# VITA-Group/UVC

Hardware: AMD Instinct MI355X
Metric: images/sec UVC Stage-1 step, DeiT-Tiny budget=0.5 (higher is better)
Workload: dtype bf16; 1 GPU; deit_tiny_patch16_224 Stage-1 UVC-train step, budget 0.5, per-GPU batch 512, 224x224x3 synthetic, soft distillation alpha 0.1, block gating on; global_batch=512, parallelism=dp1

## Files before the change

### uvc_amd/csrc/gemm.hip

```cpp
#include <type_traits>
#include "common.h"
#include "../../include/uvc_kernels.h"

template <typename T> struct Mma;
template <> struct Mma<bf16_t> {
  static constexpr int CH = 8;
  static constexpr int KSTEP = 32;
  typedef bf16x8 Frag;
  static __device__ __forceinline__ f32x4 mma(const Frag& a, const Frag& b, f32x4 c) {
    return __builtin_amdgcn_mfma_f32_16x16x32_bf16(a, b, c, 0, 0, 0);
  }
};
template <> struct Mma<float> {
  static constexpr int CH = 4;
  static constexpr int KSTEP = 16;
  typedef f32x4 Frag;
  static __device__ __forceinline__ f32x4 mma(const Frag& a, const Frag& b, f32x4 c) {
#pragma unroll
    for (int j = 0; j < 4; ++j) c = __builtin_amdgcn_mfma_f32_16x16x4f32(a[j], b[j], c, 0, 0, 0);
    return c;
  }
};

template <typename TS, typename T> struct ChunkLoad;
// ... 21 lines not shown
template <typename T> struct OutIO;
template <> struct OutIO<float> {
  static __device__ __forceinline__ void st4(float* p, f32x4 v) { *reinterpret_cast<f32x4*>(p) = v; }
  static __device__ __forceinline__ f32x4 ld4(const float* p) { return *reinterpret_cast<const f32x4*>(p); }
};
template <> struct OutIO<bf16_t> {
  static __device__ __forceinline__ void st4(bf16_t* p, f32x4 v) {
    u32x2 r; r[0] = pack_bf16x2(v[0], v[1]); r[1] = pack_bf16x2(v[2], v[3]);
    *reinterpret_cast<u32x2*>(p) = r;
  }
  static __device__ __forceinline__ f32x4 ld4(const bf16_t* p) {
    const u32x2 r = *reinterpret_cast<const u32x2*>(p);
    f32x4 v; v[0] = __uint_as_float(r[0] << 16); v[1] = __uint_as_float(r[0] & 0xffff0000u);
    v[2] = __uint_as_float(r[1] << 16); v[3] = __uint_as_float(r[1] & 0xffff0000u);
    return v;
  }
};

struct NtArgs {
  const void* A; const void* B; void* C; void* C2;
  const float* bias; const void* R; const void* R2; const void* aux; const float* dptr;
  int M, N, K, lda, ldb, ldc, ldr, ldaux;
  float alpha;
  const float* alpha_ptr;
  const float* ln_gamma; const float* ln_beta; void* ln_out; float* ln_mean; float* ln_rstd; float ln_eps;
  int no_dma;
};

template <typename TC> struct OutVec;
template <> struct OutVec<float> {
  static constexpr int VN = 4;
  static __device__ __forceinline__ void st(float* p, const float* v) { *reinterpret_cast<f32x4*>(p) = f32x4{v[0], v[1], v[2], v[3]}; }
};
template <> struct OutVec<bf16_t> {
  static constexpr int VN = 8;
  static __device__ __forceinline__ void st(bf16_t* p, const float* v) {
    u32x4 r;
    r[0] = pack_bf16x2(v[0], v[1]); r[1] = pack_bf16x2(v[2], v[3]); r[2] = pack_bf16x2(v[4], v[5]); r[3] = pack_bf16x2(v[6], v[7]);
    *reinterpret_cast<u32x4*>(p) = r;
  }
  static __device__ __forceinline__ void st_nt(bf16_t* p, const float* v) {
    u32x4 r;
    r[0] = pack_bf16x2(v[0], v[1]); r[1] = pack_bf16x2(v[2], v[3]); r[2] = pack_bf16x2(v[4], v[5]); r[3] = pack_bf16x2(v[6], v[7]);
    __builtin_nontemporal_store(r, reinterpret_cast<u32x4*>(p));
  }
};
template <typename T, int VN> __device__ __forceinline__ void load_vec(const T* p, float* v);
template <> __device__ __forceinline__ void load_vec<float, 4>(const float* p, float* v) {
  const f32x4 r = *reinterpret_cast<const f32x4*>(p); v[0] = r[0]; v[1] = r[1]; v[2] = r[2]; v[3] = r[3];
}
template <> __device__ __forceinline__ void load_vec<float, 8>(const float* p, float* v) { load_vec<float, 4>(p, v); load_vec<float, 4>(p + 4, v + 4); }
template <> __device__ __forceinline__ void load_vec<bf16_t, 8>(const bf16_t* p, float* v) {
  const u32x4 r = *reinterpret_cast<const u32x4*>(p);
#pragma unroll
  for (int e = 0; e < 4; ++e) { v[2 * e] = __uint_as_float(r[e] << 16); v[2 * e + 1] = __uint_as_float(r[e] & 0xffff0000u); }
}
template <> __device__ __forceinline__ void load_vec<bf16_t, 4>(const bf16_t* p, float* v) {
  const u32x2 r = *reinterpret_cast<const u32x2*>(p);
  v[0] = __uint_as_float(r[0] << 16); v[1] = __uint_as_float(r[0] & 0xffff0000u);
  v[2] = __uint_as_float(r[1] << 16); v[3] = __uint_as_float(r[1] & 0xffff0000u);
}

template <typename TC> struct Resid;
template <> struct Resid<float> {
  typedef u32x4 Raw4;
  static __device__ __forceinline__ Raw4 ld4(const void* base, size_t elem) { return *reinterpret_cast<const u32x4*>(reinterpret_cast<const float*>(base) + elem); }
  static __device__ __forceinline__ f32x4 f4(const Raw4& r) { return __builtin_bit_cast(f32x4, r); }
  static __device__ __forceinline__ void get(const u32x4& r, float* v) { const f32x4 f = __builtin_bit_cast(f32x4, r); v[0] = f[0]; v[1] = f[1]; v[2] = f[2]; v[3] = f[3]; }
};
template <> struct Resid<bf16_t> {
  typedef u32x2 Raw4;
  static __device__ __forceinline__ Raw4 ld4(const void* base, size_t elem) { return *reinterpret_cast<const u32x2*>(reinterpret_cast<const bf16_t*>(base) + elem); }
  static __device__ __forceinline__ f32x4 f4(const Raw4& r) {
    return f32x4{__uint_as_float(r[0] << 16), __uint_as_float(r[0] & 0xffff0000u), __uint_as_float(r[1] << 16), __uint_as_float(r[1] & 0xffff0000u)};
  }
  static __device__ __forceinline__ void get(const u32x4& r, float* v) {
#pragma unroll
    for (int e = 0; e < 4; ++e) { v[2 * e] = __uint_as_float(r[e] << 16); v[2 * e + 1] = __uint_as_float(r[e] & 0xffff0000u); }
  }
};

__device__ __forceinline__ float epi_scale_bias(float acc, float alpha, float bias) { return __builtin_fmaf(acc, alpha, bias); }
__device__ __forceinline__ float epi_gate_mix(float v, float r2, float d0, float d1) { return __builtin_fmaf(d1, v, __builtin_fmaf(d0, r2, 0.0f)); }
constexpr int EP_LD = 68;

template <bool SWZ> __device__ __forceinline__ float* stg_at(float* stg, int r, int cg) {
  return SWZ ? stg + r * 64 + ((cg ^ (r & 7)) << 2) : stg + r * EP_LD + (cg << 2);
}
template <typename TC, int EPI> __device__ __forceinline__ void nt_load_bias(const NtArgs& g, int lane, int ncol0, float* bias_v) {
  constexpr int VN = OutVec<TC>::VN, LPR = 64 / VN;
  constexpr bool has_bias = EPI == UVC_EPI_BIAS || EPI == UVC_EPI_BIAS_GELU || EPI == UVC_EPI_BIAS_GELU_OUT || EPI == UVC_EPI_BIAS_RESID ||
                            EPI == UVC_EPI_BIAS_RESID_GATE || EPI == UVC_EPI_BIAS_GELU_GRAD;
  const int n = ncol0 + (lane % LPR) * VN;
#pragma unroll
  for (int e = 0; e < VN; ++e) bias_v[e] = (has_bias && n + e < g.N) ? g.bias[n + e] : 0.f;
}
template <int NIT> struct EpiPre { u32x4 r[NIT], r2[NIT], ax[NIT]; };
template <int EPI> struct EpiOperands {
  static constexpr bool R = EPI == UVC_EPI_BIAS_RESID || EPI == UVC_EPI_BIAS_RESID_GATE, R2 = EPI == UVC_EPI_BIAS_RESID_GATE,
                        AUX = EPI == UVC_EPI_DGELU || EPI == UVC_EPI_MUL_AUX;
  static constexpr int COUNT = (R ? 1 : 0) + (R2 ? 1 : 0) + (AUX ? 1 : 0);
};
template <int EPI, int ROWS>
__device__ __forceinline__ void nt_epilogue_prefetch(const NtArgs& g, int lane, int mrow0, int ncol0, EpiPre<ROWS / 8>& P) {
  const int cc = (lane & 7) * 8, n = ncol0 + cc;
  const bool nfull = (n + 8 <= g.N) && ((g.ldc % 8) == 0);
#pragma unroll
  for (int it = 0; it < ROWS / 8; ++it) {
    const int m = mrow0 + it * 8 + (lane >> 3);
    if (m < g.M && nfull) {
      const size_t mo = (size_t)m;
      if (EpiOperands<EPI>::R && (g.ldr % 8) == 0) P.r[it] = *reinterpret_cast<const u32x4*>(reinterpret_cast<const bf16_t*>(g.R) + mo * g.ldr + n);
      if (EpiOperands<EPI>::R2 && (g.ldr % 8) == 0) P.r2[it] = *reinterpret_cast<const u32x4*>(reinterpret_cast<const bf16_t*>(g.R2) + mo * g.ldr + n);
      if (EpiOperands<EPI>::AUX && (g.ldaux % 8) == 0) P.ax[it] = *reinterpret_cast<const u32x4*>(reinterpret_cast<const bf16_t*>(g.aux) + mo * g.ldaux + n);
    }
  }
}
template <typename T, typename TC, int EPI, int ROWS = 32, bool SWZ = false, bool PRE = false>
__device__ __forceinline__ void nt_epilogue_rows(const NtArgs& g, float* stg, int lane, int mrow0, int ncol0, float alpha, float d0, float d1,
                                                 const float* bias_v, const EpiPre<ROWS / 8>* pre = nullptr) {
  static_assert(!PRE || (sizeof(TC) == 2 && sizeof(T) == 2), "operand prefetch: bf16 C and operands only");
  constexpr int VN = OutVec<TC>::VN;
  constexpr int LPR = 64 / VN;
  constexpr int RPI = 64 / LPR;
  TC* __restrict__ C = reinterpret_cast<TC*>(g.C);
  const int cc = (lane % LPR) * VN;
  const int n = ncol0 + cc;
  const bool nfull = (n + VN <= g.N) && ((g.ldc % VN) == 0);
#pragma unroll
  for (int it = 0; it < ROWS / RPI; ++it) {
    const int r = it * RPI + lane / LPR;
    const int m = mrow0 + r;
    float v[VN];
    load_vec<float, 4>(stg_at<SWZ>(stg, r, cc >> 2), v);
    if (VN == 8) load_vec<float, 4>(stg_at<SWZ>(stg, r, (cc >> 2) + 1), v + 4);
    if (m < g.M && n < g.N) {
      const size_t mo = (size_t)m;
#pragma unroll
      for (int e = 0; e < VN; ++e) v[e] = epi_scale_bias(v[e], alpha, bias_v[e]);
      if (EPI == UVC_EPI_BIAS_GELU_OUT) {
#pragma unroll
        for (int e = 0; e < VN; ++e) v[e] = Gelu<T>::f(v[e]);
      }
      if (EPI == UVC_EPI_BIAS_RESID || EPI == UVC_EPI_BIAS_RESID_GATE) {
        const TC* rp = reinterpret_cast<const TC*>(g.R) + mo * g.ldr + n;
        float rv[VN];
        if (nfull && (g.ldr % VN) == 0) { if constexpr (PRE) Resid<TC>::get(pre->r[it], rv); else load_vec<TC, VN>(rp, rv); }
        else {
#pragma unroll
          for (int e = 0; e < VN; ++e) rv[e] = (n + e < g.N) ? ElemIO<TC>::load(rp + e) : 0.f;
        }
#pragma unroll
        for (int e = 0; e < VN; ++e) v[e] += rv[e];
      }
      if (EPI == UVC_EPI_BIAS_RESID_GATE) {
        const TC* rp = reinterpret_cast<const TC*>(g.R2) + mo * g.ldr + n;
        float rv[VN];
        if (nfull && (g.ldr % VN) == 0) { if constexpr (PRE) Resid<TC>::get(pre->r2[it], rv); else load_vec<TC, VN>(rp, rv); }
        else {
#pragma unroll
          for (int e = 0; e < VN; ++e) rv[e] = (n + e < g.N) ? ElemIO<TC>::load(rp + e) : 0.f;
        }
#pragma unroll
        for (int e = 0; e < VN; ++e) v[e] = epi_gate_mix(v[e], rv[e], d0, d1);
      }
      if (EPI == UVC_EPI_DGELU || EPI == UVC_EPI_MUL_AUX) {
        const T* ap = reinterpret_cast<const T*>(g.aux) + mo * g.ldaux + n;
        float av[VN];
        if (nfull && (g.ldaux % VN) == 0) { if constexpr (PRE) Resid<TC>::get(pre->ax[it], av); else load_vec<T, VN>(ap, av); }
        else {
#pragma unroll
          for (int e = 0; e < VN; ++e) av[e] = (n + e < g.N) ? ElemIO<T>::load(ap + e) : 0.f;
        }
#pragma unroll
        for (int e = 0; e < VN; ++e) v[e] *= (EPI == UVC_EPI_MUL_AUX) ? av[e] : Gelu<T>::g(av[e]);
      }
      float u[VN];
      if (EPI == UVC_EPI_BIAS_GELU_GRAD) {
#pragma unroll
        for (int e = 0; e < VN; ++e) { float fo, go; Gelu<T>::fg(v[e], fo, go); u[e] = fo; v[e] = go; }
      }
      TC* cp = C + mo * g.ldc + n;
      if constexpr (EPI == UVC_EPI_BIAS_GELU_GRAD && sizeof(TC) == 2) { if (nfull) OutVec<TC>::st_nt(cp, v); }
      else
      if (nfull) OutVec<TC>::st(cp, v);
      if (nfull) {}
      else {
#pragma unroll
        for (int e = 0; e < VN; ++e) if (n + e < g.N) ElemIO<TC>::store(cp + e, v[e]);
      }
      if (EPI == UVC_EPI_BIAS_GELU || EPI == UVC_EPI_BIAS_GELU_GRAD) {
        TC* c2 = reinterpret_cast<TC*>(g.C2) + mo * g.ldc + n;
        if (EPI == UVC_EPI_BIAS_GELU) {
#pragma unroll
          for (int e = 0; e < VN; ++e) u[e] = Gelu<T>::f(v[e]);
        }
        if constexpr (EPI == UVC_EPI_BIAS_GELU_GRAD && sizeof(TC) == 2) { if (nfull) OutVec<TC>::st_nt(c2, u); }
        else
        if (nfull) OutVec<TC>::st(c2, u);
        if (nfull) {}
        else {
#pragma unroll
          for (int e = 0; e < VN; ++e) if (n + e < g.N) ElemIO<TC>::store(c2 + e, u[e]);
        }
      }
    }
  }
}

template <typename TA, typename T, typename TC, int EPI>
__global__ __launch_bounds__(256, 2) void k_gemm_nt(NtArgs g) {
  typedef Mma<T> MM;
  constexpr int CH = MM::CH;
  constexpr int BK = 8 * CH;
  __shared__ __attribute__((aligned(16))) char smem[(NT_BM + NT_BN) * NT_ROWB];
  char* sA = smem;
  char* sB = smem + NT_BM * NT_ROWB;
  const TA* __restrict__ A = reinterpret_cast<const TA*>(g.A);
  const T* __restrict__ B = reinterpret_cast<const T*>(g.B);
  const int tid = threadIdx.x, lane = tid & 63, w = tid >> 6;
  const int wm = w >> 1, wn = w & 1;
  const int ntn = (g.N + NT_BN - 1) / NT_BN;
  const int xcd = blockIdx.x & 7, q = blockIdx.x >> 3;
  const int bn = q % ntn, bm = (q / ntn) * 8 + xcd;
  const int m0 = bm * NT_BM, n0 = bn * NT_BN;
  if (m0 >= g.M) return;
  const int lc = tid & 7, lr = tid >> 3;

  u32x4 ra[4], rb[4];
  auto gload = [&](int k0) {
    const int kc = k0 + lc * CH;
#pragma unroll
    for (int i = 0; i < 4; ++i) {
      const int row = lr + 32 * i;
      const int m = m0 + row, n = n0 + row;
      u32x4 z = {0u, 0u, 0u, 0u};
      ra[i] = (m < g.M && kc < g.K) ? ChunkLoad<TA, T>::ld(A + (size_t)m * g.lda + kc) : z;
      rb[i] = (n < g.N && kc < g.K) ? ChunkLoad<T, T>::ld(B + (size_t)n * g.ldb + kc) : z;
    }
  };
  auto lstore = [&]() {
#pragma unroll
    for (int i = 0; i < 4; ++i) {
      const int row = lr + 32 * i;
      *reinterpret_cast<u32x4*>(sA + row * NT_ROWB + lc * 16) = ra[i];
      *reinterpret_cast<u32x4*>(sB + row * NT_ROWB + lc * 16) = rb[i];
    }
  };

  f32x4 acc[4][4];
#pragma unroll
  for (int i = 0; i < 4; ++i)
#pragma unroll
    for (int j = 0; j < 4; ++j) acc[i][j] = f32x4{0.f, 0.f, 0.f, 0.f};

  const int nk = (g.K + BK - 1) / BK;
  gload(0);
  lstore();
  __syncthreads();
  for (int kt = 0; kt < nk; ++kt) {
    if (kt + 1 < nk) gload((kt + 1) * BK);
#pragma unroll
    for (int ks = 0; ks < 2; ++ks) {
      typename MM::Frag fa[4], fb[4];
      const int coff = (ks * 4 + (lane >> 4)) * 16;
#pragma unroll
      for (int i = 0; i < 4; ++i) fa[i] = lds_frag<T>(sA + (wm * 64 + i * 16 + (lane & 15)) * NT_ROWB + coff);
#pragma unroll
      for (int j = 0; j < 4; ++j) fb[j] = lds_frag<T>(sB + (wn * 64 + j * 16 + (lane & 15)) * NT_ROWB + coff);
#pragma unroll
      for (int i = 0; i < 4; ++i)
#pragma unroll
        for (int j = 0; j < 4; ++j) acc[i][j] = MM::mma(fb[j], fa[i], acc[i][j]);
    }
    if (kt + 1 < nk) {
      __syncthreads();
      lstore();
      __syncthreads();
    }
  }

  float alpha = g.alpha;
  if (g.alpha_ptr) alpha *= *g.alpha_ptr;
  float d0 = 0.f, d1 = 1.f;
  if (EPI == UVC_EPI_BIAS_RESID_GATE) { d0 = g.dptr[0]; d1 = g.dptr[1]; }
  float* stg = reinterpret_cast<float*>(smem) + w * (32 * EP_LD);
  float bias_v[OutVec<TC>::VN];
  nt_load_bias<TC, EPI>(g, lane, n0 + wn * 64, bias_v);
  __syncthreads();
#pragma unroll
  for (int h = 0; h < 2; ++h) {
#pragma unroll
    for (int ii = 0; ii < 2; ++ii)
#pragma unroll
      for (int j = 0; j < 4; ++j)
        *reinterpret_cast<f32x4*>(stg + (ii * 16 + (lane & 15)) * EP_LD + j * 16 + (lane >> 4) * 4) = acc[2 * h + ii][j];
    __syncthreads();
    nt_epilogue_rows<T, TC, EPI>(g, stg, lane, m0 + wm * 64 + h * 32, n0 + wn * 64, alpha, d0, d1, bias_v);
    __syncthreads();
  }
}

constexpr int WS_BM = 64;

template <typename TA, typename TC, int EPI, int KT, int WS_NW, int NJ = 4>
__global__ __launch_bounds__(64 * WS_NW, (KT > 6 && WS_NW > 6) ? 1 : (NJ == 4 || KT > 6) ? 2 : 4) void k_gemm_ws(NtArgs g, int ngroups, int nslots) {
  typedef bf16_t T;
  typedef Mma<T> MM;
  constexpr int ROWB = KT * 64 + 32;
  constexpr int CPR = KT * 4;
  constexpr int NLD = (WS_BM * CPR + 64 * WS_NW - 1) / (64 * WS_NW);
  constexpr int CW = 16 * NJ, EPW = CW + 4;
  constexpr int VN = OutVec<TC>::VN, LPR = CW / VN, RPI = 64 / LPR;
  constexpr bool DYN = KT > 6;
  constexpr int IMGB = WS_BM * ROWB;
  extern __shared__ __attribute__((aligned(16))) char ws_dyn[];
  __shared__ __attribute__((aligned(16))) char sA_st[DYN ? 16 : 2 * IMGB];
  __shared__ __attribute__((aligned(16))) float sStage_st[DYN ? 4 : WS_NW * 16 * EPW];
  char* const sAb = DYN ? ws_dyn : sA_st;
  float* const sStg = DYN ? reinterpret_cast<float*>(ws_dyn + 2 * IMGB) : sStage_st;
  const int tid = threadIdx.x, lane = tid & 63, w = tid >> 6, gq = lane >> 4, li = lane & 15;
  const int L = blockIdx.x;
  const int grp = (L >> 3) % ngroups, slot = (L / (8 * ngroups)) * 8 + (L & 7);
  const int n0 = grp * CW * WS_NW + w * CW;
  const bool active = n0 < g.N;
  const TA* __restrict__ A = reinterpret_cast<const TA*>(g.A);
  const T* __restrict__ W = reinterpret_cast<const T*>(g.B);
  TC* __restrict__ C = reinterpret_cast<TC*>(g.C);
  const int ntiles = (g.M + WS_BM - 1) / WS_BM;

  typename MM::Frag bf[NJ][KT];
  if (active) {
#pragma unroll
    for (int j = 0; j < NJ; ++j)
#pragma unroll
      for (int ks = 0; ks < KT; ++ks)
        bf[j][ks] = __builtin_bit_cast(typename MM::Frag, *reinterpret_cast<const u32x4*>(W + (size_t)(n0 + j * 16 + li) * g.ldb + (ks * 4 + gq) * 8));
  }
  float alpha = g.alpha;
  if (g.alpha_ptr) alpha *= *g.alpha_ptr;
  float d0 = 0.f, d1 = 1.f;
  if (EPI == UVC_EPI_BIAS_RESID_GATE) { d0 = g.dptr[0]; d1 = g.dptr[1]; }
  const int cc = (lane % LPR) * VN;
  const int n = n0 + cc;
  float bias_v[VN];
#pragma unroll
  for (int e = 0; e < VN; ++e) bias_v[e] = 0.f;
  if (active && (EPI == UVC_EPI_BIAS || EPI == UVC_EPI_BIAS_GELU || EPI == UVC_EPI_BIAS_GELU_OUT || EPI == UVC_EPI_BIAS_RESID || EPI == UVC_EPI_BIAS_RESID_GATE ||
                 EPI == UVC_EPI_BIAS_GELU_GRAD || EPI == UVC_EPI_BIAS_GELU_GRAD_Q8)) {
#pragma unroll
    for (int e = 0; e < VN; ++e) bias_v[e] = g.bias[n + e];
  }

  u32x4 ra[NLD];
  auto gload = [&](int tile) {
    const int m0 = tile * WS_BM;
    const u32x4 z = {0u, 0u, 0u, 0u};
#pragma unroll
    for (int i = 0; i < NLD; ++i) {
      const int id = tid + 64 * WS_NW * i, row = id / CPR, c = id % CPR;
      const int m = m0 + row;
      ra[i] = (row < WS_BM && m < g.M) ? ChunkLoad<TA, T>::ld(A + (size_t)m * g.lda + c * 8) : z;
    }
  };
  auto lstore = [&](int buf) {
#pragma unroll
    for (int i = 0; i < NLD; ++i) {
      const int id = tid + 64 * WS_NW * i, row = id / CPR, c = id % CPR;
      if (row < WS_BM) *reinterpret_cast<u32x4*>(sAb + buf * IMGB + row * ROWB + c * 16) = ra[i];
    }
  };

  constexpr int IT = 16 / RPI;
  struct Epi { u32x4 r[IT]; u32x4 r2[IT]; u32x4 ax[IT]; };
  auto eload = [&](Epi& E, int tile_, int sub_) {
    if (!active) return;
#pragma unroll
    for (int it = 0; it < IT; ++it) {
      const int m = tile_ * WS_BM + sub_ * 16 + it * RPI + lane / LPR;
      const bool ok = m < g.M && tile_ < ntiles;
      const size_t mo = (size_t)(ok ? m : 0);
      if (EPI == UVC_EPI_BIAS_RESID || EPI == UVC_EPI_BIAS_RESID_GATE) E.r[it] = *reinterpret_cast<const u32x4*>(reinterpret_cast<const TC*>(g.R) + mo * g.ldr + n);
      if (EPI == UVC_EPI_BIAS_RESID_GATE) E.r2[it] = *reinterpret_cast<const u32x4*>(reinterpret_cast<const TC*>(g.R2) + mo * g.ldr + n);
      if (EPI == UVC_EPI_DGELU || EPI == UVC_EPI_MUL_AUX) E.ax[it] = *reinterpret_cast<const u32x4*>(reinterpret_cast<const T*>(g.aux) + mo * g.ldaux + n);
      if (EPI == UVC_EPI_MUL_AUX_Q8) {
        const u32x2 q = *reinterpret_cast<const u32x2*>(reinterpret_cast<const unsigned char*>(g.aux) + mo * g.ldaux + n);
        E.ax[it][0] = q[0]; E.ax[it][1] = q[1];
      }
    }
  };
  auto subtile = [&](int buf_, int m0_, int sub_, const Epi& E) {
    if (!active) return;
    float* stg = sStg + w * (16 * EPW);
    {
      typename MM::Frag fa[KT];
#pragma unroll
      for (int ks = 0; ks < KT; ++ks) fa[ks] = lds_frag<T>(sAb + buf_ * IMGB + (sub_ * 16 + li) * ROWB + (ks * 4 + gq) * 16);
#pragma unroll
      for (int j = 0; j < NJ; ++j) {
        f32x4 c = {0.f, 0.f, 0.f, 0.f};
#pragma unroll
        for (int ks = 0; ks < KT; ++ks) c = MM::mma(bf[j][ks], fa[ks], c);
        *reinterpret_cast<f32x4*>(stg + li * EPW + j * 16 + gq * 4) = c;
      }
    }
    __builtin_amdgcn_wave_barrier();
    unsigned qc[IT][2];
#pragma unroll
    for (int it = 0; it < IT; ++it) { qc[it][0] = 0u; qc[it][1] = 0u; }
#pragma unroll
    for (int it = 0; it < IT; ++it) {
      const int r = it * RPI + lane / LPR;
      const int m = m0_ + sub_ * 16 + r;
      float v[VN];
      load_vec<float, VN>(stg + r * EPW + cc, v);
      if (m < g.M) {
        const size_t mo = (size_t)m;
#pragma unroll
        for (int e = 0; e < VN; ++e) v[e] = epi_scale_bias(v[e], alpha, bias_v[e]);
        if (EPI == UVC_EPI_BIAS_RESID || EPI == UVC_EPI_BIAS_RESID_GATE) {
          float rv[VN];
          Resid<TC>::get(E.r[it], rv);
#pragma unroll
          for (int e = 0; e < VN; ++e) v[e] += rv[e];
        }
        if (EPI == UVC_EPI_BIAS_RESID_GATE) {
          float rv[VN];
          Resid<TC>::get(E.r2[it], rv);
#pragma unroll
          for (int e = 0; e < VN; ++e) v[e] = epi_gate_mix(v[e], rv[e], d0, d1);
        }
        if (EPI == UVC_EPI_DGELU) {
#pragma unroll
          for (int e = 0; e < 4; ++e) {
            v[2 * e] *= Gelu<T>::g(__uint_as_float(E.ax[it][e] << 16));
            v[2 * e + 1] *= Gelu<T>::g(__uint_as_float(E.ax[it][e] & 0xffff0000u));
          }
        }
        if (EPI == UVC_EPI_MUL_AUX) {
#pragma unroll
          for (int e = 0; e < 4; ++e) {
            v[2 * e] *= __uint_as_float(E.ax[it][e] << 16);
            v[2 * e + 1] *= __uint_as_float(E.ax[it][e] & 0xffff0000u);
          }
        }
        if constexpr (EPI == UVC_EPI_MUL_AUX_Q8) {
          static_assert(VN == 8, "q8 epilogue: bf16 C");
#pragma unroll
          for (int e = 0; e < 8; ++e)
            v[e] *= __builtin_fmaf((float)((E.ax[it][e >> 2] >> (8 * (e & 3))) & 0xffu), UVC_Q8_STEP, UVC_Q8_LO);
        }
        if (EPI == UVC_EPI_BIAS_GELU_OUT) {
#pragma unroll
          for (int e = 0; e < VN; ++e) v[e] = Gelu<T>::f(v[e]);
        }
        float u[VN];
        if (EPI == UVC_EPI_BIAS_GELU_GRAD || EPI == UVC_EPI_BIAS_GELU_GRAD_Q8) {
#pragma unroll
          for (int e = 0; e < VN; ++e) { float fo, go; Gelu<T>::fg(v[e], fo, go); u[e] = fo; v[e] = go; }
        }
        if constexpr (EPI == UVC_EPI_BIAS_GELU_GRAD_Q8) {
          static_assert(VN == 8, "q8 epilogue: bf16 C2");
          unsigned qw[2] = {0u, 0u};
#pragma unroll
          for (int e = 0; e < 8; ++e)
            qw[e >> 2] = __builtin_amdgcn_cvt_pk_u8_f32(__builtin_fmaf(v[e], 1.0f / UVC_Q8_STEP, -UVC_Q8_LO / UVC_Q8_STEP), e & 3, qw[e >> 2]);
          qc[it][0] = qw[0]; qc[it][1] = qw[1];
          OutVec<TC>::st_nt(reinterpret_cast<TC*>(g.C2) + mo * g.ldc + n, u);
        } else {
        if constexpr (EPI == UVC_EPI_BIAS_GELU_GRAD && sizeof(TC) == 2 && KT == 6) OutVec<TC>::st_nt(C + mo * g.ldc + n, v);
        else
        OutVec<TC>::st(C + mo * g.ldc + n, v);
        if (EPI == UVC_EPI_BIAS_GELU || EPI == UVC_EPI_BIAS_GELU_GRAD) {
          if (EPI == UVC_EPI_BIAS_GELU) {
#pragma unroll
            for (int e = 0; e < VN; ++e) u[e] = Gelu<T>::f(v[e]);
          }
          if constexpr (EPI == UVC_EPI_BIAS_GELU_GRAD && sizeof(TC) == 2 && KT == 6) OutVec<TC>::st_nt(reinterpret_cast<TC*>(g.C2) + mo * g.ldc + n, u);
          else
          OutVec<TC>::st(reinterpret_cast<TC*>(g.C2) + mo * g.ldc + n, u);
        }
        }
      }
    }
    if constexpr (EPI == UVC_EPI_BIAS_GELU_GRAD_Q8) {
      const bool odd = lane & 1;
      if constexpr (IT == 2) {
        static_assert(LPR == 8 && RPI == 8, "q8 epilogue: four waves x 64 columns");
        const unsigned s0 = odd ? qc[0][0] : qc[1][0], s1 = odd ? qc[0][1] : qc[1][1];
        const unsigned r0 = (unsigned)__builtin_amdgcn_mov_dpp((int)s0, 0xB1, 0xF, 0xF, true);
        const unsigned r1 = (unsigned)__builtin_amdgcn_mov_dpp((int)s1, 0xB1, 0xF, 0xF, true);
        const int m = m0_ + sub_ * 16 + (odd ? RPI : 0) + lane / LPR;
        if (m < g.M) {
          const u32x4 o = odd ? u32x4{r0, r1, qc[1][0], qc[1][1]} : u32x4{qc[0][0], qc[0][1], r0, r1};
          __builtin_nontemporal_store(o, reinterpret_cast<u32x4*>(reinterpret_cast<unsigned char*>(g.C) + (size_t)m * g.ldc + (n & ~15)));
        }
      } else {
        static_assert(IT == 1 && LPR == 4, "q8 epilogue: eight waves x 32 columns");
        const unsigned r0 = (unsigned)__builtin_amdgcn_mov_dpp((int)qc[0][0], 0xB1, 0xF, 0xF, true);
        const unsigned r1 = (unsigned)__builtin_amdgcn_mov_dpp((int)qc[0][1], 0xB1, 0xF, 0xF, true);
        const int m = m0_ + sub_ * 16 + lane / LPR;
        if (m < g.M && !odd)
          __builtin_nontemporal_store(u32x4{qc[0][0], qc[0][1], r0, r1}, reinterpret_cast<u32x4*>(reinterpret_cast<unsigned char*>(g.C) + (size_t)m * g.ldc + n));
      }
    }
    __builtin_amdgcn_wave_barrier();
  };

  int tile = slot;
  if (tile >= ntiles) return;
  Epi E0, E1;
  gload(tile);
  eload(E0, tile, 0);
  lstore(0);
  __syncthreads();
  int buf = 0;
  for (; tile < ntiles; tile += nslots) {
    const int next = tile + nslots;
    if (next < ntiles) gload(next);
    const int m0 = tile * WS_BM;
    eload(E1, tile, 1);
    subtile(buf, m0, 0, E0);
    eload(E0, tile, 2);
    subtile(buf, m0, 1, E1);
    eload(E1, tile, 3);
    subtile(buf, m0, 2, E0);
    eload(E0, next, 0);
    subtile(buf, m0, 3, E1);
    if (next < ntiles) lstore(buf ^ 1);
    __syncthreads();
    buf ^= 1;
  }
}

static bool ws_ok(const NtArgs& a, int vn) {
  return (a.K == 192 || a.K == 128) && a.N % 64 == 0 && a.ldb == a.K && a.lda % 8 == 0 && a.ldc % vn == 0 && a.ldr % vn == 0 &&
         a.ldaux % vn == 0 && a.M >= 4096;
}
template <typename TA, typename TC, int KT, int WS_NW>
static int launch_ws_epi(const NtArgs& a, int epi, hipStream_t st) {
  const int ngroups = ceil_div(a.N, 64 * WS_NW);
  const int ntiles = ceil_div(a.M, WS_BM);
#ifndef UVC_WS_WG_TOTAL
#define UVC_WS_WG_TOTAL 512
#endif
  int nslots = (UVC_WS_WG_TOTAL / ngroups) & ~7;
  if (nslots < 8) nslots = 8;
  if (nslots > ((ntiles + 7) & ~7)) nslots = (ntiles + 7) & ~7;
  const int grid = nslots * ngroups;
  if (epi == UVC_EPI_BIAS_GELU_GRAD_Q8) {
    if constexpr (sizeof(TA) == 2 && sizeof(TC) == 2 && KT == 6 && WS_NW == 4) {
      k_gemm_ws<TA, TC, UVC_EPI_BIAS_GELU_GRAD_Q8, KT, WS_NW><<<grid, 64 * WS_NW, 0, st>>>(a, ngroups, nslots);
      UVC_CHECK_LAUNCH();
      return UVC_OK;
    } else return uvc_set_error_msg(UVC_ERR_UNSUPPORTED, "uvc_gemm_nt: UVC_EPI_BIAS_GELU_GRAD_Q8 outside uvc_gemm_nt_q8_supported");
  }
#define WS_CASE(E) case E: k_gemm_ws<TA, TC, E, KT, WS_NW><<<grid, 64 * WS_NW, 0, st>>>(a, ngroups, nslots); break;
  switch (epi) {
    WS_CASE(UVC_EPI_NONE) WS_CASE(UVC_EPI_BIAS) WS_CASE(UVC_EPI_BIAS_GELU) WS_CASE(UVC_EPI_BIAS_RESID)
    WS_CASE(UVC_EPI_BIAS_RESID_GATE) WS_CASE(UVC_EPI_DGELU) WS_CASE(UVC_EPI_BIAS_GELU_OUT) WS_CASE(UVC_EPI_BIAS_GELU_GRAD) WS_CASE(UVC_EPI_MUL_AUX)
    default: return uvc_set_error_msg(UVC_ERR_ARG, "uvc_gemm_nt: unknown epilogue");
  }
#undef WS_CASE
  UVC_CHECK_LAUNCH();
  return UVC_OK;
}
static bool ws384_ok(const NtArgs& a, int epi, int vn, bool a_f32) {
  if (epi == UVC_EPI_DGELU) return false;
  if (epi == UVC_EPI_NONE && !(vn == 8 && a.N % 128 == 0 && a.N >= 512)) return false;
  return !a_f32 && a.K == 384 && a.N % 192 == 0 && a.ldb == a.K && a.lda % 8 == 0 && a.ldc % vn == 0 && a.ldr % vn == 0 && a.ldaux % vn == 0 && a.M >= 4096;
}
template <typename TC, int NW = 6>
static int launch_ws384(const NtArgs& a, int epi, hipStream_t st) {
  constexpr int KT = 12, NJ = 2;
  const int ngroups = ceil_div(a.N, 32 * NW);
  const int ntiles = ceil_div(a.M, WS_BM);
  int nslots = (256 / ngroups) & ~7;
  if (nslots < 8) nslots = 8;
  if (nslots > ((ntiles + 7) & ~7)) nslots = (ntiles + 7) & ~7;
  const int grid = nslots * ngroups;
  const int sh = 2 * WS_BM * (KT * 64 + 32) + NW * 16 * (16 * NJ + 4) * 4;
#define WS_CASE(E) case E: { \
    UVC_MAX_LDS(sh, k_gemm_ws<bf16_t, TC, E, KT, NW, NJ>); \
    k_gemm_ws<bf16_t, TC, E, KT, NW, NJ><<<grid, 64 * NW, sh, st>>>(a, ngroups, nslots); } break;
  switch (epi) {
    WS_CASE(UVC_EPI_NONE) WS_CASE(UVC_EPI_BIAS) WS_CASE(UVC_EPI_BIAS_GELU) WS_CASE(UVC_EPI_BIAS_RESID)
    WS_CASE(UVC_EPI_BIAS_RESID_GATE) WS_CASE(UVC_EPI_BIAS_GELU_OUT) WS_CASE(UVC_EPI_BIAS_GELU_GRAD) WS_CASE(UVC_EPI_MUL_AUX)
    default: return uvc_set_error_msg(UVC_ERR_ARG, "uvc_gemm_nt: unknown epilogue");
  }
#undef WS_CASE
  UVC_CHECK_LAUNCH();
  return UVC_OK;
}

template <typename TA, typename TC, int KT>
static int launch_ws_narrow(const NtArgs& a, int epi, hipStream_t st) {
  const int ngroups = ceil_div(a.N, 256);
  const int ntiles = ceil_div(a.M, WS_BM);
  int nslots = (UVC_WS_WG_TOTAL / ngroups) & ~7;
  if (nslots < 8) nslots = 8;
  if (nslots > ((ntiles + 7) & ~7)) nslots = (ntiles + 7) & ~7;
  const int grid = nslots * ngroups;
#define WS_CASE(E) case E: k_gemm_ws<TA, TC, E, KT, 8, 2><<<grid, 512, 0, st>>>(a, ngroups, nslots); break;
  switch (epi) {
    WS_CASE(UVC_EPI_DGELU) WS_CASE(UVC_EPI_MUL_AUX) WS_CASE(UVC_EPI_MUL_AUX_Q8) WS_CASE(UVC_EPI_BIAS_GELU_GRAD_Q8)
    default: return uvc_set_error_msg(UVC_ERR_ARG, "uvc_gemm_nt: epilogue");
  }
#undef WS_CASE
  UVC_CHECK_LAUNCH();
  return UVC_OK;
}
template <typename TA, typename TC>
static int launch_ws(const NtArgs& a, int epi, hipStream_t st) {
  if constexpr (sizeof(TC) == 2 && sizeof(TA) == 2) {
    if (a.N % 256 == 0 && a.K == 192 && (epi == UVC_EPI_DGELU || epi == UVC_EPI_MUL_AUX || epi == UVC_EPI_MUL_AUX_Q8)) return launch_ws_narrow<TA, TC, 6>(a, epi, st);
#ifdef UVC_FC1_NARROW
    if (a.N % 256 == 0 && a.K == 192 && epi == UVC_EPI_BIAS_GELU_GRAD_Q8) return launch_ws_narrow<TA, TC, 6>(a, epi, st);
#endif
  }
  if (epi == UVC_EPI_MUL_AUX_Q8) return uvc_set_error_msg(UVC_ERR_UNSUPPORTED, "uvc_gemm_nt: UVC_EPI_MUL_AUX_Q8 outside uvc_gemm_nt_q8_supported");
  if (a.N % 256 == 0) return a.K == 192 ? launch_ws_epi<TA, TC, 6, 4>(a, epi, st) : launch_ws_epi<TA, TC, 4, 4>(a, epi, st);
  return a.K == 192 ? launch_ws_epi<TA, TC, 6, 3>(a, epi, st) : launch_ws_epi<TA, TC, 4, 3>(a, epi, st);
}

constexpr int WN_BM = 32;

template <typename TC, int EPI, int KT>
__global__ __launch_bounds__(768) void k_gemm_wsn(NtArgs g) {
  typedef bf16_t T;
  typedef Mma<T> MM;
  constexpr int K = KT * 32, NTH = 768;
  constexpr int ROWB = K * 2 + 32, CPR = K / 8;
  constexpr int NLD = (WN_BM * CPR + NTH - 1) / NTH;
  constexpr bool RES = EPI == UVC_EPI_BIAS_RESID || EPI == UVC_EPI_BIAS_RESID_GATE;
  extern __shared__ __attribute__((aligned(16))) char smem[];
  char* sA0 = smem;
  char* sA1 = smem + WN_BM * ROWB;
  const int tid = threadIdx.x, lane = tid & 63, w = tid >> 6, gq = lane >> 4, li = lane & 15;
  const T* __restrict__ A = reinterpret_cast<const T*>(g.A);
  const T* __restrict__ W = reinterpret_cast<const T*>(g.B);
  TC* __restrict__ C = reinterpret_cast<TC*>(g.C);
  const int ntiles = (g.M + WN_BM - 1) / WN_BM;
  const int n = w * 16 + gq * 4;

  typename MM::Frag bf[KT];
#pragma unroll
  for (int ks = 0; ks < KT; ++ks)
    bf[ks] = __builtin_bit_cast(typename MM::Frag, *reinterpret_cast<const u32x4*>(W + (size_t)(w * 16 + li) * g.ldb + (ks * 4 + gq) * 8));
  float alpha = g.alpha;
  if (g.alpha_ptr) alpha *= *g.alpha_ptr;
  float d0 = 0.f, d1 = 1.f;
  if (EPI == UVC_EPI_BIAS_RESID_GATE) { d0 = g.dptr[0]; d1 = g.dptr[1]; }
  f32x4 bias4 = {0.f, 0.f, 0.f, 0.f};
  if (EPI == UVC_EPI_BIAS || RES) bias4 = *reinterpret_cast<const f32x4*>(g.bias + n);

  u32x4 ra[NLD];
  auto gload = [&](int tile) {
    const int m0 = tile * WN_BM;
    const u32x4 z = {0u, 0u, 0u, 0u};
#pragma unroll
    for (int i = 0; i < NLD; ++i) {
      const int id = tid + NTH * i, row = id / CPR, c = id % CPR;
      const int m = m0 + row;
      ra[i] = (row < WN_BM && m < g.M) ? *reinterpret_cast<const u32x4*>(A + (size_t)m * g.lda + c * 8) : z;
    }
  };
  auto lstore = [&](char* buf) {
#pragma unroll
    for (int i = 0; i < NLD; ++i) {
      const int id = tid + NTH * i, row = id / CPR, c = id % CPR;
      if (row < WN_BM) *reinterpret_cast<u32x4*>(buf + row * ROWB + c * 16) = ra[i];
    }
  };
  struct Epi { f32x4 r[2]; f32x4 r2[2]; };
  auto eload = [&](Epi& E, int tile_) {
    if (!RES) return;
#pragma unroll
    for (int s2 = 0; s2 < 2; ++s2) {
      const int m = tile_ * WN_BM + s2 * 16 + li;
      const size_t off = (m < g.M && tile_ < ntiles) ? (size_t)m * g.ldr + n : 0;
      E.r[s2] = Resid<TC>::f4(Resid<TC>::ld4(g.R, off));
      if (EPI == UVC_EPI_BIAS_RESID_GATE) E.r2[s2] = Resid<TC>::f4(Resid<TC>::ld4(g.R2, off));
    }
  };

  int tile = blockIdx.x;
  if (tile >= ntiles) return;
  Epi E, En;
  gload(tile);
  eload(E, tile);
  lstore(sA0);
  __syncthreads();
  int par = 0;
  for (; tile < ntiles; tile += gridDim.x) {
    const int next = tile + gridDim.x;
    if (next < ntiles) gload(next);
    const char* buf = par ? sA1 : sA0;
    f32x4 c0 = {0.f, 0.f, 0.f, 0.f}, c1 = {0.f, 0.f, 0.f, 0.f};
#pragma unroll
    for (int ks = 0; ks < KT; ++ks) {
      const typename MM::Frag f0 = lds_frag<T>(buf + li * ROWB + (ks * 4 + gq) * 16);
      const typename MM::Frag f1 = lds_frag<T>(buf + (16 + li) * ROWB + (ks * 4 + gq) * 16);
      c0 = MM::mma(bf[ks], f0, c0);
      c1 = MM::mma(bf[ks], f1, c1);
    }
    eload(En, next);
#pragma unroll
    for (int s2 = 0; s2 < 2; ++s2) {
      const int m = tile * WN_BM + s2 * 16 + li;
      f32x4 v = s2 ? c1 : c0;
      if (m < g.M) {
        float o[4];
#pragma unroll
        for (int e = 0; e < 4; ++e) o[e] = epi_scale_bias(v[e], alpha, bias4[e]);
        if (RES) {
#pragma unroll
          for (int e = 0; e < 4; ++e) o[e] += E.r[s2][e];
        }
        if (EPI == UVC_EPI_BIAS_RESID_GATE) {
#pragma unroll
          for (int e = 0; e < 4; ++e) o[e] = epi_gate_mix(o[e], E.r2[s2][e], d0, d1);
        }
        if (sizeof(TC) == 4) *reinterpret_cast<f32x4*>(reinterpret_cast<float*>(C) + (size_t)m * g.ldc + n) = f32x4{o[0], o[1], o[2], o[3]};
        else { u32x2 q; q[0] = pack_bf16x2(o[0], o[1]); q[1] = pack_bf16x2(o[2], o[3]); *reinterpret_cast<u32x2*>(reinterpret_cast<bf16_t*>(C) + (size_t)m * g.ldc + n) = q; }
      }
    }
    E = En;
    if (next < ntiles) lstore(par ? sA0 : sA1);
    __syncthreads();
    par ^= 1;
  }
}

template <typename TC, int EPI, int KT>
__global__ __launch_bounds__(768) void k_gemm_wsn16(NtArgs g) {
  typedef bf16_t T;
  typedef Mma<T> MM;
  constexpr int K = KT * 32, NTH = 768;
  constexpr int ROWB = K * 2 + 32, CPR = K / 8;
  constexpr int NLD = (16 * CPR + NTH - 1) / NTH;
  constexpr bool RES = EPI == UVC_EPI_BIAS_RESID || EPI == UVC_EPI_BIAS_RESID_GATE;
  extern __shared__ __attribute__((aligned(16))) char smem[];
  char* sA0 = smem;
  char* sA1 = smem + 16 * ROWB;
  const int tid = threadIdx.x, lane = tid & 63, w = tid >> 6, gq = lane >> 4, li = lane & 15;
  const T* __restrict__ A = reinterpret_cast<const T*>(g.A);
  const T* __restrict__ W = reinterpret_cast<const T*>(g.B);
  TC* __restrict__ C = reinterpret_cast<TC*>(g.C);
  const int ntiles = (g.M + 16 - 1) / 16;
  const int n = w * 16 + gq * 4;

  typename MM::Frag bf[KT];
#pragma unroll
  for (int ks = 0; ks < KT; ++ks)
    bf[ks] = __builtin_bit_cast(typename MM::Frag, *reinterpret_cast<const u32x4*>(W + (size_t)(w * 16 + li) * g.ldb + (ks * 4 + gq) * 8));
  float alpha = g.alpha;
  if (g.alpha_ptr) alpha *= *g.alpha_ptr;
  float d0 = 0.f, d1 = 1.f;
  if (EPI == UVC_EPI_BIAS_RESID_GATE) { d0 = g.dptr[0]; d1 = g.dptr[1]; }
  f32x4 bias4 = {0.f, 0.f, 0.f, 0.f};
  if (EPI == UVC_EPI_BIAS || RES) bias4 = *reinterpret_cast<const f32x4*>(g.bias + n);

  u32x4 ra[NLD];
  auto gload = [&](int tile) {
    const int m0 = tile * 16;
    const u32x4 z = {0u, 0u, 0u, 0u};
#pragma unroll
    for (int i = 0; i < NLD; ++i) {
      const int id = tid + NTH * i, row = id / CPR, c = id % CPR;
      const int m = m0 + row;
      ra[i] = (row < 16 && m < g.M) ? *reinterpret_cast<const u32x4*>(A + (size_t)m * g.lda + c * 8) : z;
    }
  };
  auto lstore = [&](char* buf) {
#pragma unroll
    for (int i = 0; i < NLD; ++i) {
      const int id = tid + NTH * i, row = id / CPR, c = id % CPR;
      if (row < 16) *reinterpret_cast<u32x4*>(buf + row * ROWB + c * 16) = ra[i];
    }
  };
  struct Epi { typename Resid<TC>::Raw4 r[1]; typename Resid<TC>::Raw4 r2[1]; };
  auto eload = [&](Epi& E, int tile_) {
    if (!RES) return;
#pragma unroll
    for (int s2 = 0; s2 < 1; ++s2) {
      const int m = tile_ * 16 + s2 * 16 + li;
      const size_t off = (m < g.M && tile_ < ntiles) ? (size_t)m * g.ldr + n : 0;
      E.r[s2] = Resid<TC>::ld4(g.R, off);
      if (EPI == UVC_EPI_BIAS_RESID_GATE) E.r2[s2] = Resid<TC>::ld4(g.R2, off);
    }
  };

  int tile = blockIdx.x;
  if (tile >= ntiles) return;
  Epi E, En;
  gload(tile);
  eload(E, tile);
  lstore(sA0);
  __syncthreads();
  int par = 0;
  for (; tile < ntiles; tile += gridDim.x) {
    const int next = tile + gridDim.x;
    if (next < ntiles) gload(next);
    const char* buf = par ? sA1 : sA0;
    f32x4 c0 = {0.f, 0.f, 0.f, 0.f};
#pragma unroll
    for (int ks = 0; ks < KT; ++ks) c0 = MM::mma(bf[ks], lds_frag<T>(buf + li * ROWB + (ks * 4 + gq) * 16), c0);
    eload(En, next);
#pragma unroll
    for (int s2 = 0; s2 < 1; ++s2) {
      const int m = tile * 16 + s2 * 16 + li;
      f32x4 v = c0;
      if (m < g.M) {
        float o[4];
#pragma unroll
        for (int e = 0; e < 4; ++e) o[e] = epi_scale_bias(v[e], alpha, bias4[e]);
        if (RES) {
          const f32x4 rv = Resid<TC>::f4(E.r[s2]);
#pragma unroll
          for (int e = 0; e < 4; ++e) o[e] += rv[e];
        }
        if (EPI == UVC_EPI_BIAS_RESID_GATE) {
          const f32x4 rv = Resid<TC>::f4(E.r2[s2]);
#pragma unroll
          for (int e = 0; e < 4; ++e) o[e] = epi_gate_mix(o[e], rv[e], d0, d1);
        }
        if (sizeof(TC) == 4) *reinterpret_cast<f32x4*>(reinterpret_cast<float*>(C) + (size_t)m * g.ldc + n) = f32x4{o[0], o[1], o[2], o[3]};
        else { u32x2 q; q[0] = pack_bf16x2(o[0], o[1]); q[1] = pack_bf16x2(o[2], o[3]); *reinterpret_cast<u32x2*>(reinterpret_cast<bf16_t*>(C) + (size_t)m * g.ldc + n) = q; }
      }
    }
    E = En;
    if (next < ntiles) lstore(par ? sA0 : sA1);
    __syncthreads();
// ... 2366 lines not shown
```

Baseline: 47230 images/sec.

## Add full-tile fast path and optional MMA/epilogue software pipeline in weight-stationary GEMM

Restructures the weight-stationary GEMM loop into mma and epilogue lambdas. A compile-time full-tile path drops per-row bounds checks for non-operand epilogues and uses 32-bit row offsets from a precomputed base pointer. An optional pipeline, UVC_WS_PIPE (off by default), overlaps the next subtile's MFMAs with the current GELU epilogue using scheduling group barriers. The fast path adds template instantiations and code size, and the 32-bit offset arithmetic assumes row offsets within a tile fit in unsigned.

```diff
diff --git a/uvc_amd/csrc/gemm.hip b/uvc_amd/csrc/gemm.hip
--- a/uvc_amd/csrc/gemm.hip
+++ b/uvc_amd/csrc/gemm.hip
@@ -347,6 +347,7 @@
 }
 
 constexpr int WS_BM = 64;
+__device__ __forceinline__ char* ws_sbase(const void* p, size_t off) { return reinterpret_cast<char*>(const_cast<void*>(p)) + off; }
 
 template <typename TA, typename TC, int EPI, int KT, int WS_NW, int NJ = 4>
 __global__ __launch_bounds__(64 * WS_NW, (KT > 6 && WS_NW > 6) ? 1 : (NJ == 4 || KT > 6) ? 2 : 4) void k_gemm_ws(NtArgs g, int ngroups, int nslots) {
@@ -417,12 +418,23 @@
   };
 
   constexpr int IT = 16 / RPI;
+#ifndef UVC_WS_PIPE
+#define UVC_WS_PIPE 0
+#endif
+  constexpr bool OPERANDS = EPI == UVC_EPI_BIAS_RESID || EPI == UVC_EPI_BIAS_RESID_GATE || EPI == UVC_EPI_DGELU || EPI == UVC_EPI_MUL_AUX || EPI == UVC_EPI_MUL_AUX_Q8;
+  constexpr bool GELU_EPI = EPI == UVC_EPI_BIAS_GELU || EPI == UVC_EPI_BIAS_GELU_OUT || EPI == UVC_EPI_BIAS_GELU_GRAD || EPI == UVC_EPI_BIAS_GELU_GRAD_Q8;
+  constexpr bool PIPE = UVC_WS_PIPE && KT == 6 && NJ == 4 && GELU_EPI;
+  constexpr bool FAST = !OPERANDS || (NJ == 2 && KT == 6 && (EPI == UVC_EPI_MUL_AUX || EPI == UVC_EPI_MUL_AUX_Q8));
+  constexpr int VPM = 6;
   struct Epi { u32x4 r[IT]; u32x4 r2[IT]; u32x4 ax[IT]; };
+  Epi E0, E1;
+  const int lrow = lane / LPR;
+  const unsigned loC = (unsigned)(lrow * g.ldc + n) * (unsigned)sizeof(TC);
   auto eload = [&](Epi& E, int tile_, int sub_) {
     if (!active) return;
 #pragma unroll
     for (int it = 0; it < IT; ++it) {
-      const int m = tile_ * WS_BM + sub_ * 16 + it * RPI + lane / LPR;
+      const int m = tile_ * WS_BM + sub_ * 16 + it * RPI + lrow;
       const bool ok = m < g.M && tile_ < ntiles;
       const size_t mo = (size_t)(ok ? m : 0);
       if (EPI == UVC_EPI_BIAS_RESID || EPI == UVC_EPI_BIAS_RESID_GATE) E.r[it] = *reinterpret_cast<const u32x4*>(reinterpret_cast<const TC*>(g.R) + mo * g.ldr + n);
@@ -434,146 +446,187 @@
       }
     }
   };
-  auto subtile = [&](int buf_, int m0_, int sub_, const Epi& E) {
-    if (!active) return;
-    float* stg = sStg + w * (16 * EPW);
-    {
-      typename MM::Frag fa[KT];
-#pragma unroll
-      for (int ks = 0; ks < KT; ++ks) fa[ks] = lds_frag<T>(sAb + buf_ * IMGB + (sub_ * 16 + li) * ROWB + (ks * 4 + gq) * 16);
-#pragma unroll
-      for (int j = 0; j < NJ; ++j) {
-        f32x4 c = {0.f, 0.f, 0.f, 0.f};
-#pragma unroll
-        for (int ks = 0; ks < KT; ++ks) c = MM::mma(bf[j][ks], fa[ks], c);
-        *reinterpret_cast<f32x4*>(stg + li * EPW + j * 16 + gq * 4) = c;
-      }
-    }
-    __builtin_amdgcn_wave_barrier();
+  float* const stg = sStg + w * (16 * EPW);
+  f32x4 acc[NJ];
+  auto mma_sub = [&](int buf_, int sub_) {
+    typename MM::Frag fa[KT];
+#pragma unroll
+    for (int ks = 0; ks < KT; ++ks) fa[ks] = lds_frag<T>(sAb + buf_ * IMGB + (sub_ * 16 + li) * ROWB + (ks * 4 + gq) * 16);
+#pragma unroll
+    for (int j = 0; j < NJ; ++j) {
+      f32x4 c = {0.f, 0.f, 0.f, 0.f};
+#pragma unroll
+      for (int ks = 0; ks < KT; ++ks) c = MM::mma(bf[j][ks], fa[ks], c);
+      if constexpr (PIPE) acc[j] = c;
+      else *reinterpret_cast<f32x4*>(stg + li * EPW + j * 16 + gq * 4) = c;
+    }
+  };
+  auto epilogue = [&](auto full_c, int m0_, int sub_, const Epi& E, const float (&v)[IT][VN]) {
+    constexpr bool FULL = decltype(full_c)::value;
     unsigned qc[IT][2];
 #pragma unroll
     for (int it = 0; it < IT; ++it) { qc[it][0] = 0u; qc[it][1] = 0u; }
 #pragma unroll
     for (int it = 0; it < IT; ++it) {
-      const int r = it * RPI + lane / LPR;
-      const int m = m0_ + sub_ * 16 + r;
-      float v[VN];
-      load_vec<float, VN>(stg + r * EPW + cc, v);
-      if (m < g.M) {
-        const size_t mo = (size_t)m;
-#pragma unroll
-        for (int e = 0; e < VN; ++e) v[e] = epi_scale_bias(v[e], alpha, bias_v[e]);
+      const int rb = m0_ + sub_ * 16 + it * RPI;
+      const bool ok = FULL || rb + lrow < g.M;
+      TC* const cp = reinterpret_cast<TC*>(ws_sbase(C, (size_t)rb * (size_t)g.ldc * sizeof(TC)) + (size_t)loC);
+      TC* const c2p = reinterpret_cast<TC*>(ws_sbase(g.C2, (size_t)rb * (size_t)g.ldc * sizeof(TC)) + (size_t)loC);
+      float vv[VN];
+      if constexpr (PIPE) {
+#pragma unroll
+        for (int e = 0; e < VN; ++e) vv[e] = v[it][e];
+      } else load_vec<float, VN>(stg + (it * RPI + lrow) * EPW + cc, vv);
+      if (ok) {
+#pragma unroll
+        for (int e = 0; e < VN; ++e) vv[e] = epi_scale_bias(vv[e], alpha, bias_v[e]);
         if (EPI == UVC_EPI_BIAS_RESID || EPI == UVC_EPI_BIAS_RESID_GATE) {
           float rv[VN];
           Resid<TC>::get(E.r[it], rv);
 #pragma unroll
-          for (int e = 0; e < VN; ++e) v[e] += rv[e];
+          for (int e = 0; e < VN; ++e) vv[e] += rv[e];
         }
         if (EPI == UVC_EPI_BIAS_RESID_GATE) {
           float rv[VN];
           Resid<TC>::get(E.r2[it], rv);
 #pragma unroll
-          for (int e = 0; e < VN; ++e) v[e] = epi_gate_mix(v[e], rv[e], d0, d1);
+          for (int e = 0; e < VN; ++e) vv[e] = epi_gate_mix(vv[e], rv[e], d0, d1);
         }
         if (EPI == UVC_EPI_DGELU) {
 #pragma unroll
           for (int e = 0; e < 4; ++e) {
-            v[2 * e] *= Gelu<T>::g(__uint_as_float(E.ax[it][e] << 16));
-            v[2 * e + 1] *= Gelu<T>::g(__uint_as_float(E.ax[it][e] & 0xffff0000u));
+            vv[2 * e] *= Gelu<T>::g(__uint_as_float(E.ax[it][e] << 16));
+            vv[2 * e + 1] *= Gelu<T>::g(__uint_as_float(E.ax[it][e] & 0xffff0000u));
           }
         }
         if (EPI == UVC_EPI_MUL_AUX) {
 #pragma unroll
           for (int e = 0; e < 4; ++e) {
-            v[2 * e] *= __uint_as_float(E.ax[it][e] << 16);
-            v[2 * e + 1] *= __uint_as_float(E.ax[it][e] & 0xffff0000u);
+            vv[2 * e] *= __uint_as_float(E.ax[it][e] << 16);
+            vv[2 * e + 1] *= __uint_as_float(E.ax[it][e] & 0xffff0000u);
           }
         }
         if constexpr (EPI == UVC_EPI_MUL_AUX_Q8) {
           static_assert(VN == 8, "q8 epilogue: bf16 C");
 #pragma unroll
           for (int e = 0; e < 8; ++e)
-            v[e] *= __builtin_fmaf((float)((E.ax[it][e >> 2] >> (8 * (e & 3))) & 0xffu), UVC_Q8_STEP, UVC_Q8_LO);
+            vv[e] *= __builtin_fmaf((float)((E.ax[it][e >> 2] >> (8 * (e & 3))) & 0xffu), UVC_Q8_STEP, UVC_Q8_LO);
         }
         if (EPI == UVC_EPI_BIAS_GELU_OUT) {
 #pragma unroll
-          for (int e = 0; e < VN; ++e) v[e] = Gelu<T>::f(v[e]);
+          for (int e = 0; e < VN; ++e) vv[e] = Gelu<T>::f(vv[e]);
         }
         float u[VN];
         if (EPI == UVC_EPI_BIAS_GELU_GRAD || EPI == UVC_EPI_BIAS_GELU_GRAD_Q8) {
 #pragma unroll
-          for (int e = 0; e < VN; ++e) { float fo, go; Gelu<T>::fg(v[e], fo, go); u[e] = fo; v[e] = go; }
+          for (int e = 0; e < VN; ++e) { float fo, go; Gelu<T>::fg(vv[e], fo, go); u[e] = fo; vv[e] = go; }
         }
         if constexpr (EPI == UVC_EPI_BIAS_GELU_GRAD_Q8) {
           static_assert(VN == 8, "q8 epilogue: bf16 C2");
           unsigned qw[2] = {0u, 0u};
 #pragma unroll
           for (int e = 0; e < 8; ++e)
-            qw[e >> 2] = __builtin_amdgcn_cvt_pk_u8_f32(__builtin_fmaf(v[e], 1.0f / UVC_Q8_STEP, -UVC_Q8_LO / UVC_Q8_STEP), e & 3, qw[e >> 2]);
+            qw[e >> 2] = __builtin_amdgcn_cvt_pk_u8_f32(__builtin_fmaf(vv[e], 1.0f / UVC_Q8_STEP, -UVC_Q8_LO / UVC_Q8_STEP), e & 3, qw[e >> 2]);
           qc[it][0] = qw[0]; qc[it][1] = qw[1];
-          OutVec<TC>::st_nt(reinterpret_cast<TC*>(g.C2) + mo * g.ldc + n, u);
+          if (ok) OutVec<TC>::st_nt(c2p, u);
         } else {
-        if constexpr (EPI == UVC_EPI_BIAS_GELU_GRAD && sizeof(TC) == 2 && KT == 6) OutVec<TC>::st_nt(C + mo * g.ldc + n, v);
+        if constexpr (EPI == UVC_EPI_BIAS_GELU_GRAD && sizeof(TC) == 2 && KT == 6) { if (ok) OutVec<TC>::st_nt(cp, vv); }
         else
-        OutVec<TC>::st(C + mo * g.ldc + n, v);
+        { if (ok) OutVec<TC>::st(cp, vv); }
         if (EPI == UVC_EPI_BIAS_GELU || EPI == UVC_EPI_BIAS_GELU_GRAD) {
           if (EPI == UVC_EPI_BIAS_GELU) {
 #pragma unroll
-            for (int e = 0; e < VN; ++e) u[e] = Gelu<T>::f(v[e]);
+            for (int e = 0; e < VN; ++e) u[e] = Gelu<T>::f(vv[e]);
           }
-          if constexpr (EPI == UVC_EPI_BIAS_GELU_GRAD && sizeof(TC) == 2 && KT == 6) OutVec<TC>::st_nt(reinterpret_cast<TC*>(g.C2) + mo * g.ldc + n, u);
+          if constexpr (EPI == UVC_EPI_BIAS_GELU_GRAD && sizeof(TC) == 2 && KT == 6) { if (ok) OutVec<TC>::st_nt(c2p, u); }
           else
-          OutVec<TC>::st(reinterpret_cast<TC*>(g.C2) + mo * g.ldc + n, u);
+          { if (ok) OutVec<TC>::st(c2p, u); }
         }
         }
       }
     }
     if constexpr (EPI == UVC_EPI_BIAS_GELU_GRAD_Q8) {
       const bool odd = lane & 1;
+      unsigned char* const qp = reinterpret_cast<unsigned char*>(ws_sbase(g.C, (size_t)(m0_ + sub_ * 16) * (size_t)g.ldc));
       if constexpr (IT == 2) {
         static_assert(LPR == 8 && RPI == 8, "q8 epilogue: four waves x 64 columns");
         const unsigned s0 = odd ? qc[0][0] : qc[1][0], s1 = odd ? qc[0][1] : qc[1][1];
         const unsigned r0 = (unsigned)__builtin_amdgcn_mov_dpp((int)s0, 0xB1, 0xF, 0xF, true);
         const unsigned r1 = (unsigned)__builtin_amdgcn_mov_dpp((int)s1, 0xB1, 0xF, 0xF, true);
-        const int m = m0_ + sub_ * 16 + (odd ? RPI : 0) + lane / LPR;
-        if (m < g.M) {
+        const int mr = (odd ? RPI : 0) + lrow;
+        if (FULL || m0_ + sub_ * 16 + mr < g.M) {
           const u32x4 o = odd ? u32x4{r0, r1, qc[1][0], qc[1][1]} : u32x4{qc[0][0], qc[0][1], r0, r1};
-          __builtin_nontemporal_store(o, reinterpret_cast<u32x4*>(reinterpret_cast<unsigned char*>(g.C) + (size_t)m * g.ldc + (n & ~15)));
+          __builtin_nontemporal_store(o, reinterpret_cast<u32x4*>(qp + (size_t)(unsigned)(mr * g.ldc + (n & ~15))));
         }
       } else {
         static_assert(IT == 1 && LPR == 4, "q8 epilogue: eight waves x 32 columns");
         const unsigned r0 = (unsigned)__builtin_amdgcn_mov_dpp((int)qc[0][0], 0xB1, 0xF, 0xF, true);
         const unsigned r1 = (unsigned)__builtin_amdgcn_mov_dpp((int)qc[0][1], 0xB1, 0xF, 0xF, true);
-        const int m = m0_ + sub_ * 16 + lane / LPR;
-        if (m < g.M && !odd)
-          __builtin_nontemporal_store(u32x4{qc[0][0], qc[0][1], r0, r1}, reinterpret_cast<u32x4*>(reinterpret_cast<unsigned char*>(g.C) + (size_t)m * g.ldc + n));
-      }
+        if ((FULL || m0_ + sub_ * 16 + lrow < g.M) && !odd)
+          __builtin_nontemporal_store(u32x4{qc[0][0], qc[0][1], r0, r1}, reinterpret_cast<u32x4*>(qp + (size_t)(unsigned)(lrow * g.ldc + n)));
+      }
+    }
+  };
+  auto subtile = [&](auto full_c, int buf_, int m0_, int sub_, const Epi& E, int nbuf, int nsub) {
+    if (!active) return;
+    if constexpr (!PIPE) mma_sub(buf_, sub_);
+    else {
+#pragma unroll
+      for (int j = 0; j < NJ; ++j) *reinterpret_cast<f32x4*>(stg + li * EPW + j * 16 + gq * 4) = acc[j];
     }
     __builtin_amdgcn_wave_barrier();
+    float v[IT][VN];
+    if constexpr (PIPE) {
+#pragma unroll
+      for (int it = 0; it < IT; ++it) load_vec<float, VN>(stg + (it * RPI + lrow) * EPW + cc, v[it]);
+      __builtin_amdgcn_wave_barrier();
+      mma_sub(nbuf, nsub);
+    }
+    epilogue(full_c, m0_, sub_, E, v);
+    if constexpr (!PIPE) __builtin_amdgcn_wave_barrier();
+    if constexpr (PIPE && decltype(full_c)::value) {
+      __builtin_amdgcn_sched_group_barrier(0x2, 2 * VPM, 0);
+#pragma unroll
+      for (int i = 0; i < NJ * KT; ++i) {
+        __builtin_amdgcn_sched_group_barrier(0x8, 1, 0);
+        __builtin_amdgcn_sched_group_barrier(0x2, VPM, 0);
+      }
+    }
+    if constexpr (PIPE) __builtin_amdgcn_sched_barrier(0);
+  };
+  auto tile_body = [&](auto full_c, int tile_, int next_, int buf_) {
+    const int m0 = tile_ * WS_BM;
+    eload(E1, tile_, 1);
+    subtile(full_c, buf_, m0, 0, E0, buf_, 1);
+    eload(E0, tile_, 2);
+    subtile(full_c, buf_, m0, 1, E1, buf_, 2);
+    eload(E1, tile_, 3);
+    subtile(full_c, buf_, m0, 2, E0, buf_, 3);
+    if constexpr (PIPE) {
+      if (next_ < ntiles) lstore(buf_ ^ 1);
+      __syncthreads();
+    }
+    eload(E0, next_, 0);
+    subtile(full_c, buf_, m0, 3, E1, buf_ ^ 1, 0);
+    if constexpr (!PIPE) {
+      if (next_ < ntiles) lstore(buf_ ^ 1);
+      __syncthreads();
+    }
   };
 
   int tile = slot;
   if (tile >= ntiles) return;
-  Epi E0, E1;
   gload(tile);
   eload(E0, tile, 0);
   lstore(0);
   __syncthreads();
+  if constexpr (PIPE) { if (active) mma_sub(0, 0); }
   int buf = 0;
   for (; tile < ntiles; tile += nslots) {
     const int next = tile + nslots;
     if (next < ntiles) gload(next);
-    const int m0 = tile * WS_BM;
-    eload(E1, tile, 1);
-    subtile(buf, m0, 0, E0);
-    eload(E0, tile, 2);
-    subtile(buf, m0, 1, E1);
-    eload(E1, tile, 3);
-    subtile(buf, m0, 2, E0);
-    eload(E0, next, 0);
-    subtile(buf, m0, 3, E1);
-    if (next < ntiles) lstore(buf ^ 1);
-    __syncthreads();
+    if (FAST && (tile + 1) * WS_BM <= g.M) tile_body(std::true_type{}, tile, next, buf);
+    else tile_body(std::false_type{}, tile, next, buf);
     buf ^= 1;
   }
 }
```

Measured after the change: 47600 images/sec, median of 6. Within noise of the previous version (+0.8%).
